# THU-LYJ-Lab/AR-Seg

Hardware: AMD Instinct MI355X
Metric: non-keyframe frames/sec (backbone+CReFF) at 512x1024 (higher is better)
Workload: dtype f32

## Files before the change

ar-seg_amd/csrc/conv_up2_c64.hip:

```cpp
#include "arseg_device.h"
#include "conv_plans.h"
#include <cmath>

namespace {

constexpr int TH = 8, TW = 16, PH = TH + 2, PW = TW + 2, NPX = PH * PW;
constexpr int PLANE = NPX * 64, BUFB = 4 * PLANE;
constexpr int BWC = PW / 2, NBLK = (PH / 2) * BWC;
constexpr int NMMA = 256, NSTAGE = 256, NT = NMMA + NSTAGE;
constexpr int MAXU = (NBLK * 16 + NSTAGE - 1) / NSTAGE;
constexpr int KT = 18;
constexpr unsigned OOB = 0x80000000u;
enum { ROLE_MMA = 0, ROLE_STAGE = 1 };

struct Up2Params {
    const float *in, *w, *scale, *bias;
    float *out;
    int H, W, in_ld, out_ld;
    int tiles_x, tiles_y, ntiles;
    int act;
    float slope;
    unsigned *range_flag;
    float range_limit;
    unsigned in_bytes, w_bytes, out_bytes;
};

struct TileRun { int first, stride, count; };
__device__ __forceinline__ TileRun tile_run(int ntiles) {
    const int G = (int)gridDim.x, b = (int)blockIdx.x, nx = G < 8 ? G : 8;
    const int xcd = b % nx, idx = b / nx, wgs = (G - xcd + nx - 1) / nx;
    const int q = ntiles / nx, r = ntiles - q * nx;
    const int start = xcd < r ? xcd * (q + 1) : r * (q + 1) + (xcd - r) * q, cnt = q + (xcd < r ? 1 : 0);
    return TileRun{start + idx, wgs, idx < cnt ? (cnt - idx + wgs - 1) / wgs : 0};
}
struct TilePos { int img, ty0, tx0; };
__device__ __forceinline__ TilePos tile_pos(const Up2Params &p, int t) {
    const int per = p.tiles_x * p.tiles_y, img = t / per, rem = t - img * per, ty = rem / p.tiles_x;
    return TilePos{img, ty * TH, (rem - ty * p.tiles_x) * TW};
}

template <int ROLE>
__device__ __forceinline__ void up2_role(const Up2Params &p, unsigned char *lds) {
    const TileRun run = tile_run(p.ntiles);
    if (run.count == 0) return;

    if constexpr (ROLE == ROLE_STAGE) {
        const int ptid = (int)threadIdx.x - NMMA;
        const __amdgpu_buffer_rsrc_t a_rsrc = __builtin_amdgcn_make_buffer_rsrc(const_cast<float *>(p.in), 0, (int)p.in_bytes, 0x00020000);
        const bool watch = p.range_flag != nullptr;
        float vmax = 0.f;
        const int h = p.H >> 1, w = p.W >> 1;
        int by[MAXU], bx[MAXU], upx[MAXU];
#pragma unroll
        for (int it = 0; it < MAXU; ++it) {
            const int b = (ptid + it * NSTAGE) >> 4;
            by[it] = b / BWC; bx[it] = b - by[it] * BWC;
            upx[it] = b < NBLK ? 2 * by[it] * PW + 2 * bx[it] : -1;
        }
        const int p16 = ptid & 15;
        u32x4 rq[MAXU][4];
        int uflag[MAXU];
        auto load_quads = [&](int t) {
            const TilePos tp = tile_pos(p, t);
#pragma unroll
            for (int it = 0; it < MAXU; ++it) {
                const int iy = (tp.ty0 >> 1) - 1 + by[it], ix = (tp.tx0 >> 1) - 1 + bx[it];
                const int ya = min(max(iy, 0), h - 1), yb = min(max(iy + 1, 0), h - 1), xa = min(max(ix, 0), w - 1), xb = min(max(ix + 1, 0), w - 1);
                const unsigned base = (unsigned)(tp.img * h) * (unsigned)w, q16 = (unsigned)p16 * 16u;
                const bool live = upx[it] >= 0;
                const unsigned o0 = live ? ((base + ya * w + xa) * p.in_ld) * 4u + q16 : OOB, o1 = live ? ((base + ya * w + xb) * p.in_ld) * 4u + q16 : OOB;
                const unsigned o2 = live ? ((base + yb * w + xa) * p.in_ld) * 4u + q16 : OOB, o3 = live ? ((base + yb * w + xb) * p.in_ld) * 4u + q16 : OOB;
                rq[it][0] = __builtin_amdgcn_raw_buffer_load_b128(a_rsrc, o0, 0, 0);
                rq[it][1] = __builtin_amdgcn_raw_buffer_load_b128(a_rsrc, o1, 0, 0);
                rq[it][2] = __builtin_amdgcn_raw_buffer_load_b128(a_rsrc, o2, 0, 0);
                rq[it][3] = __builtin_amdgcn_raw_buffer_load_b128(a_rsrc, o3, 0, 0);
                uflag[it] = ((iy >= 0 && 2 * iy + 1 < p.H) ? 1 : 0) | ((2 * iy + 2 < p.H) ? 2 : 0) | ((ix >= 0 && 2 * ix + 1 < p.W) ? 4 : 0) |
                            ((2 * ix + 2 < p.W) ? 8 : 0) | (iy < 0 ? 16 : 0) | (ix < 0 ? 32 : 0);
            }
        };
        auto stage = [&](unsigned char *buf) {
            auto put_px = [&](int px, const f32x4 v) {
                u32x2 hi, lo;
                split4(v, hi, lo);
                if (watch) vmax = fmaxf(fmaxf(vmax, fmaxf(fabsf(v[0]), fabsf(v[1]))), fmaxf(fabsf(v[2]), fabsf(v[3])));
                const int piece = p16 & 7;
                unsigned char *row = buf + (p16 >> 3) * 2 * PLANE + px * 64 + (((piece >> 1) ^ ((px >> 1) & 2)) << 4) + (piece & 1) * 8;
                *reinterpret_cast<u32x2 *>(row) = hi;
                *reinterpret_cast<u32x2 *>(row + PLANE) = lo;
            };
#pragma unroll
            for (int it = 0; it < MAXU; ++it) {
                if (upx[it] < 0) continue;
                const int f = uflag[it];
                const f32x4 q00 = __builtin_bit_cast(f32x4, rq[it][0]), q01 = __builtin_bit_cast(f32x4, rq[it][1]);
                const f32x4 q10 = __builtin_bit_cast(f32x4, rq[it][2]), q11 = __builtin_bit_cast(f32x4, rq[it][3]);
                const f32x4 r0a = 0.75f * q00 + 0.25f * q10, r0b = 0.75f * q01 + 0.25f * q11;
                const f32x4 r1a = (f & 16) ? q10 : 0.25f * q00 + 0.75f * q10, r1b = (f & 16) ? q11 : 0.25f * q01 + 0.75f * q11;
                const f32x4 z = {0.f, 0.f, 0.f, 0.f};
                const f32x4 o00 = 0.75f * r0a + 0.25f * r0b, o01 = (f & 32) ? r0b : 0.25f * r0a + 0.75f * r0b;
                const f32x4 o10 = 0.75f * r1a + 0.25f * r1b, o11 = (f & 32) ? r1b : 0.25f * r1a + 0.75f * r1b;
                put_px(upx[it], (f & 5) == 5 ? o00 : z);
                put_px(upx[it] + 1, (f & 9) == 9 ? o01 : z);
                put_px(upx[it] + PW, (f & 6) == 6 ? o10 : z);
                put_px(upx[it] + PW + 1, (f & 10) == 10 ? o11 : z);
            }
        };
        load_quads(run.first);
#pragma unroll 1
        for (int j = -1; j < run.count; ++j) {
            if (j + 1 < run.count) {
                stage(lds + ((j + 1) & 1) * BUFB);
                if (j + 2 < run.count) load_quads(run.first + (j + 2) * run.stride);
            }
            __syncthreads();
        }
        if (watch && vmax > p.range_limit) atomicOr(p.range_flag, 1u);
    } else {
        const int lane = (int)threadIdx.x & 63, slice = (int)threadIdx.x >> 6, l15 = lane & 15, kg = lane >> 4;
        h16x8 wh[KT], wl[KT];
        {
            const __amdgpu_buffer_rsrc_t b_rsrc = __builtin_amdgcn_make_buffer_rsrc(const_cast<float *>(p.w), 0, (int)p.w_bytes, 0x00020000);
            const unsigned wo = (unsigned)((slice * 16 + l15) * KT) * 128u + (unsigned)kg * 16u;
#pragma unroll
            for (int kt = 0; kt < KT; ++kt) {
                wh[kt] = __builtin_bit_cast(h16x8, __builtin_amdgcn_raw_buffer_load_b128(b_rsrc, wo + kt * 128, 0, 0));
                wl[kt] = __builtin_bit_cast(h16x8, __builtin_amdgcn_raw_buffer_load_b128(b_rsrc, wo + kt * 128 + 64, 0, 0));
            }
        }
        const int c0 = slice * 16 + kg * 4;
        float sc[4], bi[4];
#pragma unroll
        for (int r = 0; r < 4; ++r) { sc[r] = p.scale ? p.scale[c0 + r] : 1.0f; bi[r] = p.bias ? p.bias[c0 + r] : 0.0f; }
        const ArsegAct ea = arseg_act(p.act, p.slope);
        const u32x4 o_rsrc = make_rsrc(p.out, p.out_bytes);
        unsigned swz[8];
#pragma unroll
        for (int j = 0; j < 8; ++j) swz[j] = (unsigned)(l15 * 64 + ((kg ^ (((l15 + j) >> 1) & 2)) << 4));

        __syncthreads();
#pragma unroll 1
        for (int j = 0; j < run.count; ++j) {
            const unsigned char *buf = lds + (j & 1) * BUFB;
            const unsigned char *pj[8];
#pragma unroll
            for (int i = 0; i < 8; ++i) pj[i] = buf + swz[i];
            f32x4 acc[TH];
#pragma unroll
            for (int mf = 0; mf < TH; ++mf) acc[mf] = f32x4{0.f, 0.f, 0.f, 0.f};
            h16x8 fh[2][2], fl[2][2];
            auto frags = [&](int g, h16x8 (&h)[2], h16x8 (&l)[2]) {
                const int ck = g / 36, tap = (g % 36) >> 2;
#pragma unroll
                for (int u = 0; u < 2; ++u) {
                    const int C = (2 * (g & 3) + u + tap / 3) * PW + tap % 3;
                    h[u] = *reinterpret_cast<const h16x8 *>(pj[C & 7] + 2 * ck * PLANE + C * 64);
                    l[u] = *reinterpret_cast<const h16x8 *>(pj[C & 7] + (2 * ck + 1) * PLANE + C * 64);
                }
            };
            frags(0, fh[0], fl[0]);
#pragma unroll
            for (int g = 0; g < 72; ++g) {
                if (g + 1 < 72) frags(g + 1, fh[(g + 1) & 1], fl[(g + 1) & 1]);
                const int kt = 2 * ((g % 36) >> 2) + g / 36;
#pragma unroll
                for (int u = 0; u < 2; ++u) {
                    const int mf = 2 * (g & 3) + u;
                    acc[mf] = __builtin_amdgcn_mfma_f32_16x16x32_f16(wh[kt], fl[g & 1][u], acc[mf], 0, 0, 0);
                    acc[mf] = __builtin_amdgcn_mfma_f32_16x16x32_f16(wl[kt], fh[g & 1][u], acc[mf], 0, 0, 0);
                    acc[mf] = __builtin_amdgcn_mfma_f32_16x16x32_f16(wh[kt], fh[g & 1][u], acc[mf], 0, 0, 0);
                }
                __builtin_amdgcn_sched_group_barrier(0x100, 4, 0);
                __builtin_amdgcn_sched_group_barrier(0x008, 6, 0);
                __builtin_amdgcn_sched_barrier(0);
            }
            const TilePos tp = tile_pos(p, run.first + j * run.stride);
            const int ox = tp.tx0 + l15;
#pragma unroll
            for (int mf = 0; mf < TH; ++mf) {
                const int oy = tp.ty0 + mf;
                f32x4 v;
#pragma unroll
                for (int r = 0; r < 4; ++r) v[r] = arseg_act_apply(acc[mf][r] * sc[r] + bi[r], ea);
                const unsigned m = ((unsigned)tp.img * (unsigned)p.H + (unsigned)oy) * (unsigned)p.W + (unsigned)ox;
                store16_buf(__builtin_bit_cast(u32x4, v), o_rsrc, (oy < p.H && ox < p.W) ? (m * (unsigned)p.out_ld + (unsigned)c0) * 4u : OOB);
            }
            __syncthreads();
        }
    }
}

__global__ __launch_bounds__(NT) void conv_up2_c64_kernel(const Up2Params p) {
    extern __shared__ __attribute__((aligned(16))) unsigned char up2_smem[];
    if (threadIdx.x < NMMA) up2_role<ROLE_MMA>(p, up2_smem);
    else up2_role<ROLE_STAGE>(p, up2_smem);
}

}

extern "C" int arseg_conv_up2_c64_fwd(const arseg_conv_desc *d, const float *in, const float *w_packed, const float *scale, const float *bias, float *out,
                                      int max_wgs, arseg_stream_t stream) {
    if (!d) return ARSEG_EINVAL;
    if (d->N <= 0 || d->H <= 0 || d->W <= 0 || max_wgs < 0) return ARSEG_EINVAL;
    if (!conv_up2_c64_shape(d)) return ARSEG_EUNSUPPORTED;
    if (d->in_ld < 64 || (d->in_ld & 3) || d->out_ld < 64) return ARSEG_EINVAL;
    if (d->out_ld & 3) return ARSEG_EUNSUPPORTED;
    if (d->act != ARSEG_ACT_NONE && d->act != ARSEG_ACT_RELU && d->act != ARSEG_ACT_PRELU && d->act != ARSEG_ACT_SIGMOID) return ARSEG_EINVAL;
    ARSEG_CHECK_PTR(in); ARSEG_CHECK_PTR(w_packed); ARSEG_CHECK_PTR(out);
    if (!ARSEG_ALIGNED16(in) || !ARSEG_ALIGNED16(w_packed)) return ARSEG_EINVAL;
    if (!ARSEG_ALIGNED16(out)) return ARSEG_EUNSUPPORTED;
    void *rf = d->range_flag;
    if (rf && (reinterpret_cast<uintptr_t>(rf) & 3)) return ARSEG_EINVAL;
    const long long ib = conv_up2_c64_in_bytes(d), ob = conv_up2_c64_out_bytes(d);
    if ((long long)d->N * d->H * d->W > (1ll << 30) || ib >= (1ll << 31) || ob >= (1ll << 31)) return ARSEG_EUNSUPPORTED;
    Up2Params p;
    p.in = in; p.w = w_packed; p.scale = scale; p.bias = bias; p.out = out;
    p.H = d->H; p.W = d->W; p.in_ld = d->in_ld; p.out_ld = d->out_ld;
    p.tiles_x = arseg_cdiv(d->W, TW); p.tiles_y = arseg_cdiv(d->H, TH); p.ntiles = d->N * p.tiles_x * p.tiles_y;
    p.act = d->act; p.slope = d->prelu_slope;
    p.range_flag = reinterpret_cast<unsigned *>(rf);
    p.range_limit = d->range_limit > 0.0f ? d->range_limit : 65504.0f;
    p.in_bytes = (unsigned)ib; p.w_bytes = (unsigned)(64 * KT * 128); p.out_bytes = (unsigned)ob;
    hipStream_t hs = arseg_stream(stream);
    static ArsegSmemAttr attr;
    if (int e = arseg_allow_smem(attr, reinterpret_cast<const void *>(conv_up2_c64_kernel), 2 * BUFB)) return e;
    const int cus = arseg_cu_count(max_wgs), grid = p.ntiles < cus ? p.ntiles : cus;
    hipLaunchKernelGGL(conv_up2_c64_kernel, dim3(grid), dim3(NT), 2 * BUFB, hs, p);
    return arseg_launch_status();
}
```

Before: 2384.

## Prefetch next tile before staging and use lighter barriers in up2 conv

The staging warps now double-buffer global loads into registers (rn/nflag) and issue the next tile's loads before staging the current one, so the load latency overlaps the upsample math. __syncthreads is replaced with a custom barrier that waits only on LDS counters, so outstanding stores and loads are not drained at each tile boundary. The epilogue hoists address computation, uses fma, and specialises on activation type. The bilinear mix is rewritten with fma and a swapped operand order for the first iteration, which may change rounding. The extra register arrays raise pressure on the staging threads.

```diff
diff --git a/ar-seg_amd/csrc/conv_up2_c64.hip b/ar-seg_amd/csrc/conv_up2_c64.hip
--- a/ar-seg_amd/csrc/conv_up2_c64.hip
+++ b/ar-seg_amd/csrc/conv_up2_c64.hip
@@ -1,6 +1,7 @@
 #include "arseg_device.h"
 #include "conv_plans.h"
 #include <cmath>
+#include <type_traits>
 
 namespace {
 
@@ -39,6 +40,14 @@
     return TilePos{img, ty * TH, (rem - ty * p.tiles_x) * TW};
 }
 
+__device__ __forceinline__ void tile_barrier() {
+    asm volatile("s_waitcnt lgkmcnt(0)" ::: "memory");
+    __builtin_amdgcn_sched_barrier(0);
+    __builtin_amdgcn_s_barrier();
+    __builtin_amdgcn_sched_barrier(0);
+    asm volatile("" ::: "memory");
+}
+
 template <int ROLE>
 __device__ __forceinline__ void up2_role(const Up2Params &p, unsigned char *lds) {
     const TileRun run = tile_run(p.ntiles);
@@ -58,8 +67,8 @@
             upx[it] = b < NBLK ? 2 * by[it] * PW + 2 * bx[it] : -1;
         }
         const int p16 = ptid & 15;
-        u32x4 rq[MAXU][4];
-        int uflag[MAXU];
+        u32x4 rq[MAXU][4], rn[MAXU][4];
+        int uflag[MAXU], nflag[MAXU];
         auto load_quads = [&](int t) {
             const TilePos tp = tile_pos(p, t);
 #pragma unroll
@@ -70,14 +79,15 @@
                 const bool live = upx[it] >= 0;
                 const unsigned o0 = live ? ((base + ya * w + xa) * p.in_ld) * 4u + q16 : OOB, o1 = live ? ((base + ya * w + xb) * p.in_ld) * 4u + q16 : OOB;
                 const unsigned o2 = live ? ((base + yb * w + xa) * p.in_ld) * 4u + q16 : OOB, o3 = live ? ((base + yb * w + xb) * p.in_ld) * 4u + q16 : OOB;
-                rq[it][0] = __builtin_amdgcn_raw_buffer_load_b128(a_rsrc, o0, 0, 0);
-                rq[it][1] = __builtin_amdgcn_raw_buffer_load_b128(a_rsrc, o1, 0, 0);
-                rq[it][2] = __builtin_amdgcn_raw_buffer_load_b128(a_rsrc, o2, 0, 0);
-                rq[it][3] = __builtin_amdgcn_raw_buffer_load_b128(a_rsrc, o3, 0, 0);
-                uflag[it] = ((iy >= 0 && 2 * iy + 1 < p.H) ? 1 : 0) | ((2 * iy + 2 < p.H) ? 2 : 0) | ((ix >= 0 && 2 * ix + 1 < p.W) ? 4 : 0) |
+                rn[it][0] = __builtin_amdgcn_raw_buffer_load_b128(a_rsrc, o0, 0, 0);
+                rn[it][1] = __builtin_amdgcn_raw_buffer_load_b128(a_rsrc, o1, 0, 0);
+                rn[it][2] = __builtin_amdgcn_raw_buffer_load_b128(a_rsrc, o2, 0, 0);
+                rn[it][3] = __builtin_amdgcn_raw_buffer_load_b128(a_rsrc, o3, 0, 0);
+                nflag[it] = ((iy >= 0 && 2 * iy + 1 < p.H) ? 1 : 0) | ((2 * iy + 2 < p.H) ? 2 : 0) | ((ix >= 0 && 2 * ix + 1 < p.W) ? 4 : 0) |
                             ((2 * ix + 2 < p.W) ? 8 : 0) | (iy < 0 ? 16 : 0) | (ix < 0 ? 32 : 0);
             }
         };
+        auto mix = [](float ca, const f32x4 a, float cb, const f32x4 b) { return __builtin_elementwise_fma(f32x4{ca, ca, ca, ca}, a, cb * b); };
         auto stage = [&](unsigned char *buf) {
             auto put_px = [&](int px, const f32x4 v) {
                 u32x2 hi, lo;
@@ -94,11 +104,12 @@
                 const int f = uflag[it];
                 const f32x4 q00 = __builtin_bit_cast(f32x4, rq[it][0]), q01 = __builtin_bit_cast(f32x4, rq[it][1]);
                 const f32x4 q10 = __builtin_bit_cast(f32x4, rq[it][2]), q11 = __builtin_bit_cast(f32x4, rq[it][3]);
-                const f32x4 r0a = 0.75f * q00 + 0.25f * q10, r0b = 0.75f * q01 + 0.25f * q11;
-                const f32x4 r1a = (f & 16) ? q10 : 0.25f * q00 + 0.75f * q10, r1b = (f & 16) ? q11 : 0.25f * q01 + 0.75f * q11;
+                const f32x4 r0a = mix(0.75f, q00, 0.25f, q10), r0b = mix(0.75f, q01, 0.25f, q11);
+                const f32x4 r1a = (f & 16) ? q10 : mix(0.25f, q00, 0.75f, q10), r1b = (f & 16) ? q11 : mix(0.25f, q01, 0.75f, q11);
                 const f32x4 z = {0.f, 0.f, 0.f, 0.f};
-                const f32x4 o00 = 0.75f * r0a + 0.25f * r0b, o01 = (f & 32) ? r0b : 0.25f * r0a + 0.75f * r0b;
-                const f32x4 o10 = 0.75f * r1a + 0.25f * r1b, o11 = (f & 32) ? r1b : 0.25f * r1a + 0.75f * r1b;
+                const f32x4 o00 = mix(0.75f, r0a, 0.25f, r0b), o01 = (f & 32) ? r0b : mix(0.25f, r0a, 0.75f, r0b);
+                const f32x4 o10 = it ? mix(0.75f, r1a, 0.25f, r1b) : mix(0.25f, r1b, 0.75f, r1a);
+                const f32x4 o11 = (f & 32) ? r1b : (it ? mix(0.25f, r1a, 0.75f, r1b) : mix(0.75f, r1b, 0.25f, r1a));
                 put_px(upx[it], (f & 5) == 5 ? o00 : z);
                 put_px(upx[it] + 1, (f & 9) == 9 ? o01 : z);
                 put_px(upx[it] + PW, (f & 6) == 6 ? o10 : z);
@@ -109,10 +120,16 @@
 #pragma unroll 1
         for (int j = -1; j < run.count; ++j) {
             if (j + 1 < run.count) {
+#pragma unroll
+                for (int it = 0; it < MAXU; ++it) {
+                    uflag[it] = nflag[it];
+#pragma unroll
+                    for (int q = 0; q < 4; ++q) rq[it][q] = rn[it][q];
+                }
+                if (j + 2 < run.count) load_quads(run.first + (j + 2) * run.stride);
                 stage(lds + ((j + 1) & 1) * BUFB);
-                if (j + 2 < run.count) load_quads(run.first + (j + 2) * run.stride);
-            }
-            __syncthreads();
+            }
+            tile_barrier();
         }
         if (watch && vmax > p.range_limit) atomicOr(p.range_flag, 1u);
     } else {
@@ -137,7 +154,8 @@
 #pragma unroll
         for (int j = 0; j < 8; ++j) swz[j] = (unsigned)(l15 * 64 + ((kg ^ (((l15 + j) >> 1) & 2)) << 4));
 
-        __syncthreads();
+        __builtin_amdgcn_s_waitcnt(0x0F70);
+        tile_barrier();
 #pragma unroll 1
         for (int j = 0; j < run.count; ++j) {
             const unsigned char *buf = lds + (j & 1) * BUFB;
@@ -147,6 +165,11 @@
             f32x4 acc[TH];
 #pragma unroll
             for (int mf = 0; mf < TH; ++mf) acc[mf] = f32x4{0.f, 0.f, 0.f, 0.f};
+            const TilePos tp = tile_pos(p, run.first + j * run.stride);
+            const int ox = tp.tx0 + l15;
+            const unsigned o0 = ((((unsigned)tp.img * (unsigned)p.H + (unsigned)tp.ty0) * (unsigned)p.W + (unsigned)ox) * (unsigned)p.out_ld + (unsigned)c0) * 4u;
+            unsigned o0v = o0, oy0 = (unsigned)tp.ty0, ostep = (unsigned)p.W * (unsigned)p.out_ld * 4u;
+            asm volatile("" : "+v"(o0v), "+s"(oy0), "+s"(ostep));
             h16x8 fh[2][2], fl[2][2];
             auto frags = [&](int g, h16x8 (&h)[2], h16x8 (&l)[2]) {
                 const int ck = g / 36, tap = (g % 36) >> 2;
@@ -173,19 +196,28 @@
                 __builtin_amdgcn_sched_group_barrier(0x008, 6, 0);
                 __builtin_amdgcn_sched_barrier(0);
             }
-            const TilePos tp = tile_pos(p, run.first + j * run.stride);
-            const int ox = tp.tx0 + l15;
-#pragma unroll
-            for (int mf = 0; mf < TH; ++mf) {
-                const int oy = tp.ty0 + mf;
-                f32x4 v;
-#pragma unroll
-                for (int r = 0; r < 4; ++r) v[r] = arseg_act_apply(acc[mf][r] * sc[r] + bi[r], ea);
-                const unsigned m = ((unsigned)tp.img * (unsigned)p.H + (unsigned)oy) * (unsigned)p.W + (unsigned)ox;
-                store16_buf(__builtin_bit_cast(u32x4, v), o_rsrc, (oy < p.H && ox < p.W) ? (m * (unsigned)p.out_ld + (unsigned)c0) * 4u : OOB);
-            }
-            __syncthreads();
-        }
+            auto epilogue = [&](auto kind) {
+#pragma unroll
+                for (int mf = 0; mf < TH; ++mf) {
+                    f32x4 v;
+#pragma unroll
+                    for (int r = 0; r < 4; ++r) {
+                        const float y = __builtin_fmaf(acc[mf][r], sc[r], bi[r]);
+                        if constexpr (kind() == 2) v[r] = arseg_act_apply(y, ea);
+                        else {
+                            const float t = y >= 0.0f ? y : y * ea.slope;
+                            v[r] = (kind() == 1 && y < 0.0f) ? 0.0f : t;
+                        }
+                    }
+                    store16_buf(__builtin_bit_cast(u32x4, v), o_rsrc, ((int)oy0 + mf < p.H && ox < p.W) ? o0v + (unsigned)mf * ostep : OOB);
+                }
+            };
+            if (ea.sigmoid) epilogue(std::integral_constant<int, 2>{});
+            else if (ea.relu) epilogue(std::integral_constant<int, 1>{});
+            else epilogue(std::integral_constant<int, 0>{});
+            tile_barrier();
+        }
+        asm volatile("s_waitcnt vmcnt(0)" ::: "memory");
     }
 }
 
```

New measurement: 2397 (median of 6 runs). About the same (+0.5%).
